# VainF/Diff-Pruning

Measured on NVIDIA H100. Metric: taylor_score_unet_fwd_bwd_passes_per_sec, higher is better.
Workload: dtype f32

## Files before the change

diff-pruning_b200/_lib.py:

```python
from __future__ import annotations

import ctypes as C
import os

_HERE = os.path.dirname(os.path.abspath(__file__))
LIB_PATH = os.path.join(_HERE, "libdpb200.so")

i32, i64, f32, u64, vp = C.c_int32, C.c_int64, C.c_float, C.c_uint64, C.c_void_p


class ConvArgs(C.Structure):
    _fields_ = [(n, i32) for n in ("N", "H", "W", "C", "P", "Q", "K", "R", "S", "stride", "pad_t", "pad_l", "flags",
                                   "splits")] + [
        ("x", vp), ("ldx", i64), ("y", vp), ("ldy", i64), ("w", vp), ("w_tc_hi", vp), ("w_tc_lo", vp), ("bias", vp), ("rowadd", vp),
        ("ld_rowadd", i64), ("residual", vp), ("ld_res", i64), ("workspace", vp), ("amax_x", vp), ("amax_y", vp), ("amax_w", vp), ("amax_out", vp), ("bias_ws", vp)]


class WgradReduceArgs(C.Structure):
    _fields_ = [(n, i32) for n in ("K", "C", "R", "S", "splits")] + [
        ("workspace", vp), ("dw", vp), ("w", vp), ("score_out", vp), ("score_in", vp), ("bias_ws", vp), ("db", vp)]


class GemmArgs(C.Structure):
    _fields_ = [("M", i32), ("N", i32), ("Kd", i32), ("batch", i32),
                ("A", vp), ("a_rs", i64), ("a_cs", i64), ("a_bs", i64),
                ("B", vp), ("b_rs", i64), ("b_cs", i64), ("b_bs", i64),
                ("C", vp), ("ldc", i64), ("c_bs", i64), ("alpha", f32), ("accumulate", i32)]


class GemmNtArgs(C.Structure):
    _fields_ = [("batch", i32), ("H", i32), ("W", i32), ("Kg", i32), ("N", i32), ("A", vp), ("ld_a", i64), ("b_hi", vp),
                ("b_lo", vp), ("C", vp), ("ldc", i64), ("alpha", f32), ("amax_a", vp), ("amax_b", vp), ("amax_out", vp)]


class GnArgs(C.Structure):
    _fields_ = [("N", i32), ("HW", i32), ("C", i32), ("G", i32), ("eps", f32), ("silu", i32),
                ("x", vp), ("ldx", i64), ("y", vp), ("ldy", i64), ("gamma", vp), ("beta", vp), ("mean", vp),
                ("rstd", vp), ("dy", vp), ("lddy", i64), ("dx", vp), ("lddx", i64), ("dx_add", vp), ("ldadd", i64),
                ("dx_add2", vp), ("ldadd2", i64), ("dgamma", vp), ("dbeta", vp), ("workspace", vp),
                ("dropout_p", f32), ("dropout_seed", u64), ("dropout_seed_dev", vp), ("y_bf16", vp), ("ldyb", i64),
                ("amax_y", vp), ("amax_dx", vp), ("fin", vp)]


class ConvBf16Args(C.Structure):
    _fields_ = [(n, i32) for n in ("N", "H", "W", "C", "P", "Q", "K", "R", "S", "stride", "pad_t", "pad_l", "flags", "splits")] + [
        ("x_bf16", vp), ("ldx", i64), ("dy_bf16", vp), ("lddy", i64), ("out", vp), ("ld_out", i64), ("w_bf16", vp), ("bias", vp),
        ("rowadd", vp), ("ld_rowadd", i64), ("residual", vp), ("ld_res", i64), ("workspace", vp)]


class TaylorArgs(C.Structure):
    _fields_ = [("O", i32), ("I", i32), ("RS", i32), ("w", vp), ("dw", vp), ("out_signed", vp), ("out_abs", vp),
                ("out_sq", vp), ("in_signed", vp), ("in_abs", vp), ("in_sq", vp)]


class SsimArgs(C.Structure):
    _fields_ = [("x", vp), ("y", vp), ("format", i32), ("N", i32), ("C", i32), ("H", i32), ("W", i32), ("win_size", i32),
                ("win", C.c_double * 11), ("c1", C.c_double), ("c2", C.c_double), ("ssim_nc", vp), ("sse_n", vp)]


class AdamArgs(C.Structure):
    _fields_ = [("n", i64), ("p", vp), ("g", vp), ("m", vp), ("v", vp), ("ema", vp), ("sumsq", vp),
                ("max_norm", C.c_double), ("lr", C.c_double), ("beta1", C.c_double), ("beta2", C.c_double),
                ("eps", C.c_double), ("ema_decay", C.c_double),
                ("step", i32), ("grad_scale", f32), ("step_scalars", vp)]


_SIGS = {
    "dp_version": (C.c_int, []),
    "dp_strerror": (C.c_char_p, [C.c_int]),
    "dp_last_cuda_error": (C.c_int, []),
    "dp_launch_count": (i64, []),
    "dp_tc_available": (C.c_int, []),
    "dp_tc_weight_row": (C.c_int, [C.c_int]),
    "dp_conv2d_fprop": (C.c_int, [C.POINTER(ConvArgs), vp]),
    "dp_conv2d_dgrad": (C.c_int, [C.POINTER(ConvArgs), vp]),
    "dp_conv2d_wgrad": (C.c_int, [C.POINTER(ConvArgs), vp]),
    "dp_conv_splitk_workspace_floats": (i64, [C.POINTER(ConvArgs), C.c_int]),
    "dp_conv2d_wgrad_reduce": (C.c_int, [C.POINTER(WgradReduceArgs), vp]),
    "dp_pack_conv_weight": (C.c_int, [vp, i32, i32, i32, i32, vp, vp, vp]),
    "dp_pack_conv_weight_tc": (C.c_int, [vp, i32, i32, i32, i32, vp, vp, vp, vp, vp, vp]),
    "dp_amax": (C.c_int, [vp, i64, i64, i32, vp, vp]),
    "dp_zero_u32": (C.c_int, [vp, i64, vp]),
    "dp_bf16_available": (C.c_int, []),
    "dp_bf16_weight_row": (C.c_int, [C.c_int]),
    "dp_bf16_wgrad_ctile": (C.c_int, [C.c_int]),
    "dp_conv2d_fprop_bf16": (C.c_int, [C.POINTER(ConvBf16Args), vp]),
    "dp_conv2d_dgrad_bf16": (C.c_int, [C.POINTER(ConvBf16Args), vp]),
    "dp_conv2d_wgrad_bf16": (C.c_int, [C.POINTER(ConvBf16Args), vp]),
    "dp_conv_bf16_eligible": (C.c_int, [C.POINTER(ConvBf16Args), C.c_int]),
    "dp_cvt_bf16": (C.c_int, [vp, i64, i64, i32, vp, i64, vp]),
    "dp_pack_conv_weight_bf16": (C.c_int, [vp, i32, i32, i32, i32, vp, vp, vp]),
    "dp_gemm_batched": (C.c_int, [C.POINTER(GemmArgs), vp]),
    "dp_gemm_nt_tc": (C.c_int, [C.POINTER(GemmNtArgs), vp]),
    "dp_split_h3": (C.c_int, [vp, i64, i64, i32, i32, i32, i32, vp, vp, vp, vp]),
    "dp_transpose_batched": (C.c_int, [vp, vp, i32, i32, i32, vp]),
    "dp_softmax_fwd": (C.c_int, [vp, vp, i64, i32, vp]),
    "dp_softmax_bwd": (C.c_int, [vp, vp, vp, i64, i32, vp, vp]),
    "dp_groupnorm_workspace_bytes": (C.c_size_t, [i32, i32, i32, i32]),
    "dp_groupnorm_fwd": (C.c_int, [C.POINTER(GnArgs), vp]),
    "dp_groupnorm_bwd": (C.c_int, [C.POINTER(GnArgs), vp]),
    "dp_groupnorm_bwd_param": (C.c_int, [C.POINTER(GnArgs), vp]),
    "dp_silu_fwd": (C.c_int, [vp, vp, i64, vp]),
    "dp_silu_bwd": (C.c_int, [vp, vp, vp, i64, i32, vp]),
    "dp_geglu_fwd": (C.c_int, [vp, i64, vp, i64, i64, i32, vp]),
    "dp_geglu_bwd": (C.c_int, [vp, i64, vp, i64, vp, i64, i64, i32, vp]),
    "dp_timestep_embedding": (C.c_int, [vp, vp, vp, i32, i32, i32, vp]),
    "dp_add_noise": (C.c_int, [vp, vp, vp, vp, vp, i32, i32, i32, i32, i32, i64, vp]),
    "dp_nchw_to_nhwc": (C.c_int, [vp, vp, i64, i32, i32, i32, i32, vp]),
    "dp_nhwc_to_nchw": (C.c_int, [vp, i64, vp, i32, i32, i32, i32, i32, vp]),
    "dp_mse_partials": (i64, [i64]),
    "dp_mse_loss_grad": (C.c_int, [vp, vp, vp, i64, f32, f32, vp, vp, vp]),
    "dp_upsample2x_fwd": (C.c_int, [vp, i64, vp, i64, i32, i32, i32, i32, vp]),
    "dp_upsample2x_bwd": (C.c_int, [vp, i64, vp, i64, i32, i32, i32, i32, i32, vp]),
    "dp_colsum": (C.c_int, [vp, i64, i64, i32, i64, vp, i64, i32, vp]),
    "dp_add_views": (C.c_int, [vp, i64, vp, i64, vp, i64, i64, i32, vp]),
    "dp_copy_rows": (C.c_int, [vp, i64, vp, i64, i64, i32, vp]),
    "dp_taylor_reduce": (C.c_int, [C.POINTER(TaylorArgs), vp]),
    "dp_sumsq_partials": (i64, [i64]),
    "dp_sumsq": (C.c_int, [vp, i64, vp, vp, vp]),
    "dp_adam_clip_ema": (C.c_int, [C.POINTER(AdamArgs), vp]),
    "dp_ddim_step": (C.c_int, [vp, vp, vp, vp, i64, f32, f32, f32, f32, f32, f32, vp]),
    "dp_ddim_cfg_step": (C.c_int, [vp, i64, vp, vp, vp, vp, i64, vp, i32, i32, i32, i32, i32, f32, f32, f32, f32, f32, f32, vp]),
    "dp_scale": (C.c_int, [vp, i64, f32, vp]),
    "dp_fid_input": (C.c_int, [vp, i32, i32, i32, i32, i32, vp, i64, i32, i32, i32, i32, vp, vp]),
    "dp_pool3x3": (C.c_int, [vp, i64, vp, i64, i32, i32, i32, i32, i32, i32, i32, vp, vp]),
    "dp_global_mean": (C.c_int, [vp, i64, vp, i64, i32, i32, i32, i32, vp]),
    "dp_feature_moments": (C.c_int, [vp, i64, i64, i32, vp, vp, vp, vp]),
    "dp_ssim": (C.c_int, [C.POINTER(SsimArgs), vp]),
    "dp_vq_quantize": (C.c_int, [vp, i32, i32, i32, i32, f32, vp, i32, i32, vp, i64, vp, vp]),
    "dp_decode_images": (C.c_int, [vp, i64, i32, i32, i32, i32, vp, vp, vp]),
# ... 34 lines not shown
```

diff-pruning_b200/csrc/conv_tc.cu:

```cuda
#include <cuda.h>
#include <cuda_fp16.h>
#include "common.cuh"
#include "sm90.cuh"
#include "sm90_host.cuh"

namespace {
using namespace sm90;

constexpr int BM = 128, BK = 64;
constexpr int A_BYTES = BM * 32 * 4;

struct TcParams {
  int Nimg, H, W;
  int Nout;
  int kchunks;
  int bw, bh, bn, tiles_w, tiles_h;
  float* y; long long ldy;
  const float* bias;
  const float* rowadd; long long ld_rowadd;
  const float* residual; long long ld_res;
  int accumulate;
  int vec4;
  int ntaps;
  signed char dh[9], dw[9], wt[9];
  int os, oa, ob, Ho, Wo;
  int in_stride;
  float alpha;
  int b_from_img;
  const uint32_t* amax_a;
  const uint32_t* amax_b;
  uint32_t* amax_out;
  int ksplit, it_per_split;
  float* ws; long long ws_split_stride; int ws_ld;
  const float* gx; long long gldx;
  int gH, gW, gC, gQ, gPQ, gS, gstride, gpad_t, gpad_l, gM;
  int relu;
};

__device__ __forceinline__ int amax_exponent(const uint32_t* slot) {
  const int E = (int)((__ldg(slot) >> 23) & 0xFFu);
  return min(max(E, 14), 254);
}
__device__ __forceinline__ float scale_up(int E) { return __uint_as_float((uint32_t)(267 - E) << 23); }
__device__ __forceinline__ float scale_dn(int E) { return __uint_as_float((uint32_t)(E - 13) << 23); }
constexpr float LO_SCALE = 2048.f, LO_UNSCALE = 1.f / 2048.f;
__device__ __forceinline__ void split2(float a, float b, uint32_t& h, uint32_t& l) {
  const __half2 hh = __floats2half2_rn(a, b);
  const float2 hf = __half22float2(hh);
  const __half2 ll = __floats2half2_rn((a - hf.x) * LO_SCALE, (b - hf.y) * LO_SCALE);
  h = *reinterpret_cast<const uint32_t*>(&hh);
  l = *reinterpret_cast<const uint32_t*>(&ll);
}
__device__ __forceinline__ void split1(float v, __half& h, __half& l) {
  h = __float2half_rn(v);
  l = __float2half_rn((v - __half2float(h)) * LO_SCALE);
}

constexpr int PS_STAGES = 3, PS_BN = 128;
constexpr int PS_B_BYTES = PS_BN * BK * 2;
constexpr int PS_STAGE_BYTES = 2 * A_BYTES + 2 * PS_B_BYTES;

template <bool ANY>
__global__ void __launch_bounds__(THREADS, 1)
conv_tc_ps_kernel(const __grid_constant__ CUtensorMap mapA, const __grid_constant__ CUtensorMap mapBh,
                  const __grid_constant__ CUtensorMap mapBl, const TcParams p, const int tiles_m, const int total_tiles) {
  const int total_work = total_tiles * p.ksplit;
  extern __shared__ uint8_t smem_raw[];
  const uint32_t raw = smem_u32(smem_raw);
  const uint32_t pad_to = ((raw + 1023u) & ~1023u) - raw;
  uint8_t* smem = smem_raw + pad_to;
  const uint32_t sbase = raw + pad_to;
  const uint32_t bar0 = sbase + PS_STAGES * PS_STAGE_BYTES;
  auto full_bar = [&](int s) { return bar0 + 8u * s; };
  auto empty_bar = [&](int s) { return bar0 + 8u * (PS_STAGES + s); };
  const int wg = threadIdx.x >> 7, tid = threadIdx.x & 127;
  if (threadIdx.x == 0) {
    for (int s = 0; s < PS_STAGES; ++s) { mbar_init(full_bar(s), ANY ? 1 + 128 : 1); mbar_init(empty_bar(s), 8); }
    mbar_init_fence();
  }
  __syncthreads();
  const int iters_per_tile = p.ntaps * p.kchunks;

  auto tile_coords = [&](int tile, int& q0, int& p0, int& n0, int& nblk) {
    nblk = tile / tiles_m;
    const int tile_m = tile - nblk * tiles_m;
    const int tw = tile_m % p.tiles_w;
    const int th = (tile_m / p.tiles_w) % p.tiles_h;
    const int tn = tile_m / (p.tiles_w * p.tiles_h);
    q0 = tw * p.bw; p0 = th * p.bh; n0 = tn * p.bn;
  };

  if (wg == 0) {
    setmaxnreg_dec<40>();
    if constexpr (ANY) {
      const int t = threadIdx.x;
      if (t == 0) { prefetch_map(&mapBh); prefetch_map(&mapBl); }
      const uint32_t sw = (uint32_t)(t & 7);
      uint32_t g = 0;
      for (int wi = blockIdx.x; wi < total_work; wi += gridDim.x) {
        const int tile = wi % total_tiles, it0 = (wi / total_tiles) * p.it_per_split, it1 = min(iters_per_tile, it0 + p.it_per_split);
        const int nblk = tile / tiles_m, m = (tile - nblk * tiles_m) * BM + t;
        const bool mv = m < p.gM;
        const int n = mv ? m / p.gPQ : 0, rem = m - n * p.gPQ, pq = rem / p.gQ;
        const int hb = pq * p.gstride - p.gpad_t, wb = (rem - pq * p.gQ) * p.gstride - p.gpad_l;
        const float* xn = p.gx + (long long)n * p.gH * p.gW * p.gldx;
        for (int it = it0; it < it1; ++it, ++g) {
          const int s = g % PS_STAGES;
          const uint32_t ph = (g / PS_STAGES) & 1u;
          mbar_wait(empty_bar(s), ph ^ 1u);
          const int tap = it / p.kchunks, kc = it - tap * p.kchunks;
          const int r = tap / p.gS, h = hb + r, w = wb + (tap - r * p.gS);
          const uint32_t st = sbase + s * PS_STAGE_BYTES;
          if (t == 0) {
            mbar_expect_tx(full_bar(s), 2 * PS_B_BYTES);
            tma_load_3d(st + 2 * A_BYTES, &mapBh, full_bar(s), kc * BK, nblk * PS_BN, tap);
            tma_load_3d(st + 2 * A_BYTES + PS_B_BYTES, &mapBl, full_bar(s), kc * BK, nblk * PS_BN, tap);
          }
          const bool v = mv && h >= 0 && h < p.gH && w >= 0 && w < p.gW;
          const int cleft = v ? p.gC - kc * BK : 0;
          const float* src = v ? xn + ((long long)h * p.gW + w) * p.gldx + kc * BK : p.gx;
#pragma unroll
          for (int j = 0; j < 16; ++j) {
            const int nb = min(max(cleft - 4 * j, 0), 4) * 4;
            cp_async16(st + (j >> 3) * A_BYTES + t * 128 + ((((uint32_t)j & 7u) ^ sw) << 4), nb ? src + 4 * j : p.gx, (uint32_t)nb);
          }
          cp_async_mbar_arrive(full_bar(s));
        }
      }
      return;
    }
    if (threadIdx.x == 0) {
      prefetch_map(&mapA); prefetch_map(&mapBh); prefetch_map(&mapBl);
      uint32_t g = 0;
      for (int wi = blockIdx.x; wi < total_work; wi += gridDim.x) {
        const int tile = wi % total_tiles, it0 = (wi / total_tiles) * p.it_per_split, it1 = min(iters_per_tile, it0 + p.it_per_split);
        int q0, p0, n0, nblk;
        tile_coords(tile, q0, p0, n0, nblk);
        for (int it = it0; it < it1; ++it, ++g) {
          const int s = g % PS_STAGES;
          const uint32_t ph = (g / PS_STAGES) & 1u;
          mbar_wait(empty_bar(s), ph ^ 1u);
          mbar_expect_tx(full_bar(s), PS_STAGE_BYTES);
          const int tap = it / p.kchunks, kc = it - tap * p.kchunks;
          const uint32_t st = sbase + s * PS_STAGE_BYTES;
          const int aw = q0 * p.in_stride + p.dw[tap], ah = p0 * p.in_stride + p.dh[tap];
          tma_load_4d(st, &mapA, full_bar(s), kc * BK, aw, ah, n0);
          tma_load_4d(st + A_BYTES, &mapA, full_bar(s), kc * BK + 32, aw, ah, n0);
          const int tapb = p.b_from_img ? n0 : p.wt[tap];
          tma_load_3d(st + 2 * A_BYTES, &mapBh, full_bar(s), kc * BK, nblk * PS_BN, tapb);
          tma_load_3d(st + 2 * A_BYTES + PS_B_BYTES, &mapBl, full_bar(s), kc * BK, nblk * PS_BN, tapb);
        }
      }
    }
    return;
  }
  setmaxnreg_inc<232>();
  const int c = wg - 1;
  const int warp = tid >> 5, lane = tid & 31;
  const uint32_t frag_row = (uint32_t)(64 * c + 16 * warp + (lane >> 2)) * 128 + 8 * (lane & 1);
  const uint32_t fsw = (uint32_t)(lane >> 2), fj = (uint32_t)((lane & 3) >> 1);
  const float sa = scale_up(amax_exponent(p.amax_a));
  const float f1 = scale_dn(amax_exponent(p.amax_a)), f2 = scale_dn(amax_exponent(p.amax_b)) * p.alpha;
  auto fin = [&](float main, float corr) { return fmaf(corr, LO_UNSCALE, main) * f1 * f2; };
  float amax = 0.f;
  uint32_t g = 0;
  for (int wi = blockIdx.x; wi < total_work; wi += gridDim.x) {
    const int tile = wi % total_tiles, it0 = (wi / total_tiles) * p.it_per_split, it1 = min(iters_per_tile, it0 + p.it_per_split);
    float acc[64], cor[64];
    uint32_t fh[2][4], fl[2][4];
    int prev_s = 0;
    for (int it = it0; it < it1; ++it, ++g) {
      const int s = g % PS_STAGES;
      const uint32_t ph = (g / PS_STAGES) & 1u;
      mbar_wait(full_bar(s), ph);
      const uint8_t* stp = smem + s * PS_STAGE_BYTES + frag_row;
      const uint32_t bst = sbase + s * PS_STAGE_BYTES + 2 * A_BYTES;
#pragma unroll
      for (int k = 0; k < BK / 16; ++k) {
        uint32_t (&ah)[4] = fh[k & 1];
        uint32_t (&al)[4] = fl[k & 1];
        const uint8_t* a = stp + (k >> 1) * A_BYTES;
        const uint32_t pos = ((4u * (k & 1) + fj) ^ fsw) << 4;
        const float2 v0 = *reinterpret_cast<const float2*>(a + pos), v1 = *reinterpret_cast<const float2*>(a + 1024 + pos);
        const float2 v2 = *reinterpret_cast<const float2*>(a + (pos ^ 32u)), v3 = *reinterpret_cast<const float2*>(a + 1024 + (pos ^ 32u));
        split2(v0.x * sa, v0.y * sa, ah[0], al[0]);
        split2(v1.x * sa, v1.y * sa, ah[1], al[1]);
        split2(v2.x * sa, v2.y * sa, ah[2], al[2]);
        split2(v3.x * sa, v3.y * sa, ah[3], al[3]);
        const uint64_t b_hi = desc_k(bst + k * 32), b_lo = desc_k(bst + PS_B_BYTES + k * 32);
        const uint32_t first = (it > it0 || k > 0) ? 1u : 0u;
        wgmma_fence();
        wgmma_f16_n128_rs<0>(acc, ah, b_hi, first);
        wgmma_f16_n128_rs<0>(cor, ah, b_lo, first);
        wgmma_f16_n128_rs<0>(cor, al, b_hi, 1u);
        wgmma_commit();
        wgmma_wait<1>();
        if (k == 0 && it > it0 && lane == 0) mbar_arrive(empty_bar(prev_s));
      }
      prev_s = s;
    }
    wgmma_wait<0>();
    fence_regs(acc); fence_regs(cor);
    if (lane == 0) mbar_arrive(empty_bar(prev_s));

    int q0, p0, n0, nblk;
    tile_coords(tile, q0, p0, n0, nblk);
#pragma unroll
    for (int i = 0; i < 2; ++i) {
      const int row = 64 * c + 16 * warp + (lane >> 2) + 8 * i;
      const int cb = 2 * (lane & 3);
      if (p.ksplit > 1) {
        float* wrow = p.ws + (long long)(wi / total_tiles) * p.ws_split_stride + ((long long)(tile - nblk * tiles_m) * BM + row) * p.ws_ld + nblk * PS_BN;
#pragma unroll
        for (int j = 0; j < 16; ++j)
          *reinterpret_cast<float2*>(wrow + 8 * j + cb) =
              make_float2(fin(acc[4 * j + 2 * i], cor[4 * j + 2 * i]), fin(acc[4 * j + 2 * i + 1], cor[4 * j + 2 * i + 1]));
        continue;
      }
      const int w_l = row % p.bw, h_l = (row / p.bw) % p.bh, n_l = row / (p.bw * p.bh);
      const int img = n0 + n_l;
      if (img >= p.Nimg) continue;
      if constexpr (ANY) { if (q0 + w_l >= p.Wo) continue; }
      const long long m = ((long long)img * p.Ho + ((p0 + h_l) * p.os + p.oa)) * p.Wo + ((q0 + w_l) * p.os + p.ob);
// ... 240 lines not shown
#pragma unroll
    for (int k = 0; k < WG_KPIX / 16; ++k) {
      const uint64_t b_hi = desc_mn(st + 4 * WG_BLK + k * 2048, WG_BLK), b_lo = desc_mn(st + 6 * WG_BLK + k * 2048, WG_BLK);
      const uint32_t first = (it > 0 || k > 0) ? 1u : 0u;
      wgmma_f16_n128_rs<1>(acc, fah[k], b_hi, first);
      wgmma_f16_n128_rs<1>(cor, fah[k], b_lo, first);
      wgmma_f16_n128_rs<1>(cor, fal[k], b_hi, 1u);
    }
    wgmma_commit();
    wgmma_wait<1>();
    if (it > 0 && lane == 0) mbar_arrive(empty_bar(prev_s));
    prev_s = s;
  };
  uint32_t fah0[4][4], fal0[4][4], fah1[4][4], fal1[4][4];
  int it = 0;
  for (; it + 1 < num_iters; it += 2) {
    stage(fah0, fal0, it);
    stage(fah1, fal1, it + 1);
  }
  if (it < num_iters) stage(fah0, fal0, it);
  wgmma_wait<0>();
  fence_regs(acc); fence_regs(cor);
#pragma unroll
  for (int i = 0; i < 2; ++i) {
    bsum[i] += __shfl_xor_sync(0xffffffffu, bsum[i], 1);
    bsum[i] += __shfl_xor_sync(0xffffffffu, bsum[i], 2);
  }
  const float f1 = scale_dn(Ey), f2 = scale_dn(Ex);
  const long long TC_ = (long long)T * p.C;
#pragma unroll
  for (int i = 0; i < 2; ++i) {
    const int kout = kt * 128 + 64 * c + 16 * warp + (lane >> 2) + 8 * i;
    if (kout >= p.K) continue;
    if (p.bias_ws && tap == 0 && ct == 0 && (lane & 3) == 0) p.bias_ws[(long long)blockIdx.y * p.K + kout] = bsum[i];
    float* wrow = p.ws + ((long long)blockIdx.y * p.K + kout) * TC_ + (long long)tap * p.C;
#pragma unroll
    for (int j = 0; j < 16; ++j)
#pragma unroll
      for (int e = 0; e < 2; ++e) {
        const int col = ct * 128 + 8 * j + 2 * (lane & 3) + e;
        if (col < p.C) wrow[col] = num_iters ? fmaf(cor[4 * j + 2 * i + e], LO_UNSCALE, acc[4 * j + 2 * i + e]) * f1 * f2 : 0.f;
      }
  }
}

constexpr int PS_SMEM = PS_STAGES * PS_STAGE_BYTES + 2048;
constexpr int WG_SMEM = WG_STAGES * WG_STAGE_BYTES + 2048;

static int wrow(int c) { return c > 64 ? ((c + 63) & ~63) : ((c + 7) & ~7); }

int tc_init() {
  static const int ok = [] {
    const bool set = runtime().encode &&
        cudaFuncSetAttribute(conv_tc_ps_kernel<false>, cudaFuncAttributeMaxDynamicSharedMemorySize, PS_SMEM) == cudaSuccess &&
        cudaFuncSetAttribute(conv_tc_ps_kernel<true>, cudaFuncAttributeMaxDynamicSharedMemorySize, PS_SMEM) == cudaSuccess &&
        cudaFuncSetAttribute(wgrad_tc_kernel, cudaFuncAttributeMaxDynamicSharedMemorySize, WG_SMEM) == cudaSuccess;
    (void)cudaGetLastError();
    return set ? 1 : 0;
  }();
  return ok;
}

static int pick_ksplit(int tiles, int iters, int& it_per_split) {
  it_per_split = iters;
  const int sms = runtime().num_sms;
  if (tiles * 2 > sms || iters < 8) return 1;
  int ks = sms / tiles;
  if (ks > iters / 4) ks = iters / 4;
  if (ks > 16) ks = 16;
  if (ks < 2) return 1;
  it_per_split = (iters + ks - 1) / ks;
  return (iters + it_per_split - 1) / it_per_split;
}

struct TcPlan { int bw, bh, bn, tiles_w, tiles_h, tiles_m, n_tiles, ksplit, it_per_split; long long ws_floats; };
int plan_tc(const ConvGemm& g, bool flat, bool split, TcPlan& pl) {
  if (!tc_init()) return DP_ERR_UNSUPPORTED;
  if (flat) { pl.bw = BM; pl.bh = 1; pl.bn = 1; }
  else if (!pick_box(BM, g.H, g.W, pl.bw, pl.bh, pl.bn)) return DP_ERR_UNSUPPORTED;
  pl.tiles_w = (g.W + pl.bw - 1) / pl.bw; pl.tiles_h = g.H / pl.bh;
  pl.tiles_m = pl.tiles_w * pl.tiles_h * ((g.N + pl.bn - 1) / pl.bn);
  pl.n_tiles = (g.Nout + PS_BN - 1) / PS_BN;
  const int iters = g.taps.n * ((g.Kg + BK - 1) / BK);
  pl.ksplit = 1; pl.it_per_split = iters;
  if (split) pl.ksplit = pick_ksplit(pl.tiles_m * pl.n_tiles, iters, pl.it_per_split);
  pl.ws_floats = pl.ksplit > 1 ? (long long)pl.ksplit * pl.tiles_m * BM * pl.n_tiles * PS_BN : 0;
  return DP_OK;
}

struct TcLaunch {
  const float* act; long long ld_act; const uint32_t* amax_a;
  const void* w_hi; const void* w_lo; const uint32_t* amax_b; int T; int ldb = -1;
  float* out; long long ld_out;
  const float* bias = nullptr; const float* rowadd = nullptr; long long ld_rowadd = 0; const float* residual = nullptr; long long ld_res = 0;
  int accumulate = 0;
  float* ws = nullptr;
  uint32_t* amax_out = nullptr;
  float alpha = 1.0f;
  int b_from_img = 0;
  const dp_conv_args* gather = nullptr;
};

TcLaunch conv_launch(const dp_conv_args* a, bool dgrad) {
  TcLaunch l{};
  l.act = (const float*)(dgrad ? a->y : a->x); l.ld_act = dgrad ? a->ldy : a->ldx; l.amax_a = dgrad ? a->amax_y : a->amax_x;
  l.w_hi = a->w_tc_hi; l.w_lo = a->w_tc_lo; l.amax_b = a->amax_w; l.T = a->R * a->S;
  l.out = (float*)(dgrad ? a->x : a->y); l.ld_out = dgrad ? a->ldx : a->ldy;
  if (!dgrad) { l.bias = a->bias; l.rowadd = a->rowadd; l.ld_rowadd = a->ld_rowadd; l.residual = a->residual; l.ld_res = a->ld_res; }
  l.accumulate = (a->flags & DP_CONV_ACCUMULATE) ? 1 : 0;
  l.ws = a->workspace; l.amax_out = a->amax_out;
  return l;
}

int launch_tc(const ConvGemm& g, const TcLaunch& l, cudaStream_t st) {
  const bool any = l.gather != nullptr, split = l.ws && !l.b_from_img;
  TcPlan pl;
  if (plan_tc(g, any, split, pl) != DP_OK) return DP_ERR_UNSUPPORTED;
  if (!l.w_hi || !l.w_lo || !l.amax_a || !l.amax_b) return DP_ERR_UNSUPPORTED;
  if (l.ld_act % 4 || ((uintptr_t)l.act & 15) || ((uintptr_t)l.w_hi & 15) || ((uintptr_t)l.w_lo & 15)) return DP_ERR_UNSUPPORTED;
  if (l.b_from_img && pl.bn != 1) return DP_ERR_UNSUPPORTED;
  CUtensorMap mA, mBh, mBl;
  if (!any) {
    const int s = g.in_stride;
    const cuuint64_t Hin = (cuuint64_t)g.H * s, Win = (cuuint64_t)g.W * s;
    cuuint64_t dims[4] = {(cuuint64_t)g.Kg, Win, Hin, (cuuint64_t)g.N};
    cuuint64_t str[3] = {(cuuint64_t)l.ld_act * 4, Win * l.ld_act * 4, Hin * Win * l.ld_act * 4};
    cuuint32_t box[4] = {32u, (cuuint32_t)(pl.bw * s), (cuuint32_t)(pl.bh * s), (cuuint32_t)pl.bn};
    if (box[1] > 256 || box[2] > 256) return DP_ERR_UNSUPPORTED;
    if (!encode_map(&mA, CU_TENSOR_MAP_DATA_TYPE_FLOAT32, l.act, 4, dims, str, box, s)) return DP_ERR_UNSUPPORTED;
  }
  {
    const cuuint64_t Kp = (cuuint64_t)(l.ldb < 0 ? wrow(g.Kg) : l.ldb);
    if (Kp % 8) return DP_ERR_UNSUPPORTED;
    cuuint64_t dims[3] = {Kp, (cuuint64_t)g.Nout, (cuuint64_t)l.T};
    cuuint64_t str[2] = {Kp * 2, (cuuint64_t)g.Nout * Kp * 2};
    cuuint32_t box[3] = {(cuuint32_t)BK, (cuuint32_t)PS_BN, 1};
    if (!encode_map(&mBh, CU_TENSOR_MAP_DATA_TYPE_FLOAT16, l.w_hi, 3, dims, str, box) ||
        !encode_map(&mBl, CU_TENSOR_MAP_DATA_TYPE_FLOAT16, l.w_lo, 3, dims, str, box)) return DP_ERR_UNSUPPORTED;
  }
  TcParams p{};
  p.Nimg = g.N; p.H = g.H; p.W = g.W; p.Nout = g.Nout;
  p.ntaps = g.taps.n;
  for (int i = 0; i < 9; ++i) { p.dh[i] = g.taps.dh[i]; p.dw[i] = g.taps.dw[i]; p.wt[i] = g.taps.wt[i]; }
  p.os = g.os; p.oa = g.oa; p.ob = g.ob; p.Ho = g.Ho; p.Wo = g.Wo;
  p.alpha = l.alpha; p.b_from_img = l.b_from_img; p.in_stride = g.in_stride; p.amax_a = l.amax_a; p.amax_b = l.amax_b; p.amax_out = l.amax_out;
  p.kchunks = (g.Kg + BK - 1) / BK;
  p.bw = pl.bw; p.bh = pl.bh; p.bn = pl.bn; p.tiles_w = pl.tiles_w; p.tiles_h = pl.tiles_h;
  p.y = l.out; p.ldy = l.ld_out; p.bias = l.bias; p.rowadd = l.rowadd; p.ld_rowadd = l.ld_rowadd; p.residual = l.residual; p.ld_res = l.ld_res;
  p.accumulate = l.accumulate;
  p.vec4 = (al16(l.out, l.ld_out) && al16(l.bias, 0) && al16(l.rowadd, l.ld_rowadd) && al16(l.residual, l.ld_res)) ? 1 : 0;
  p.ksplit = pl.ksplit; p.it_per_split = pl.it_per_split;
  if (split) { p.ws = l.ws; p.ws_ld = pl.n_tiles * PS_BN; p.ws_split_stride = (long long)pl.tiles_m * BM * p.ws_ld; }
  if (any) {
    const dp_conv_args* a = l.gather;
    p.gx = l.act; p.gldx = l.ld_act; p.gH = a->H; p.gW = a->W; p.gC = a->C; p.gQ = a->Q; p.gPQ = a->P * a->Q; p.gS = a->S;
    p.gstride = a->stride; p.gpad_t = a->pad_t; p.gpad_l = a->pad_l; p.gM = g.W; p.relu = (a->flags & DP_CONV_RELU) ? 1 : 0;
  }
  const int sms = runtime().num_sms, total = pl.tiles_m * pl.n_tiles, work = total * p.ksplit, ctas = work < sms ? work : sms;
  if (any) conv_tc_ps_kernel<true><<<ctas, THREADS, PS_SMEM, st>>>(mBh, mBh, mBl, p, pl.tiles_m, total);
  else conv_tc_ps_kernel<false><<<ctas, THREADS, PS_SMEM, st>>>(mA, mBh, mBl, p, pl.tiles_m, total);
  if (p.ksplit > 1) {
    const int rc = dp_check_launch();
    if (rc) return rc;
    const long long items = (any ? (long long)g.W : (long long)pl.tiles_m * BM) * ((g.Nout + 3) / 4);
    long long blocks = (items + 255) / 256;
    if (blocks > sms * 8) blocks = sms * 8;
    if (any) splitk_flat_epilogue_kernel<<<(int)blocks, 256, 0, st>>>(p);
    else splitk_epilogue_kernel<<<(int)blocks, 256, 0, st>>>(p, pl.tiles_m);
  }
  return dp_check_launch();
}

__global__ void pack_tc_kernel(const float* __restrict__ w, int K, int C, int RS, int Cp, int Kp, __half* __restrict__ kc_hi,
                               __half* __restrict__ kc_lo, __half* __restrict__ ck_hi, __half* __restrict__ ck_lo,
                               const uint32_t* __restrict__ amax) {
  const float sw = scale_up(amax_exponent(amax));
  const long long na = (long long)RS * K * Cp, nb = (long long)RS * C * Kp;
  const long long total = na > nb ? na : nb;
  for (long long i = blockIdx.x * (long long)blockDim.x + threadIdx.x; i < total; i += (long long)gridDim.x * blockDim.x) {
    if (i < na && kc_hi) {
      int c = (int)(i % Cp); long long t = i / Cp; int k = (int)(t % K), tap = (int)(t / K);
      split1(c < C ? w[((long long)k * C + c) * RS + tap] * sw : 0.f, kc_hi[i], kc_lo[i]);
    }
    if (i < nb && ck_hi) {
      int k = (int)(i % Kp); long long t = i / Kp; int c = (int)(t % C), tap = (int)(t / C);
      split1(k < K ? w[((long long)k * C + c) * RS + tap] * sw : 0.f, ck_hi[i], ck_lo[i]);
    }
  }
}
__global__ void split_h3_rows_kernel(const float* __restrict__ x, long long ld, long long bs, int rows, int cols, int pitch, int vec,
                                     __half* __restrict__ hi, __half* __restrict__ lo, const uint32_t* __restrict__ amax) {
  const float sx = scale_up(amax_exponent(amax));
  const int groups = pitch >> 3;
  const long long total = (long long)rows * groups;
  const float* xb = x + (long long)blockIdx.y * bs;
  __half* hb = hi + (long long)blockIdx.y * rows * pitch;
  __half* lb = lo + (long long)blockIdx.y * rows * pitch;
  for (long long i = blockIdx.x * 256ll + threadIdx.x; i < total; i += (long long)gridDim.x * 256) {
    const long long r = i / groups;
    const int c0 = (int)(i - r * groups) << 3;
    const float* src = xb + r * ld + c0;
    float v[8];
    if (vec && c0 + 8 <= cols) {
      const float4 a = __ldg(reinterpret_cast<const float4*>(src)), b = __ldg(reinterpret_cast<const float4*>(src + 4));
      v[0] = a.x; v[1] = a.y; v[2] = a.z; v[3] = a.w; v[4] = b.x; v[5] = b.y; v[6] = b.z; v[7] = b.w;
    } else {
#pragma unroll
      for (int j = 0; j < 8; ++j) v[j] = (c0 + j < cols) ? __ldg(src + j) : 0.f;
    }
    uint4 h, l;
    split2(v[0] * sx, v[1] * sx, h.x, l.x); split2(v[2] * sx, v[3] * sx, h.y, l.y);
    split2(v[4] * sx, v[5] * sx, h.z, l.z); split2(v[6] * sx, v[7] * sx, h.w, l.w);
    *reinterpret_cast<uint4*>(hb + r * pitch + c0) = h;
// ... 187 lines not shown
  if (!tc_init()) return DP_ERR_UNSUPPORTED;
  if (!box_geometry(a) || a->splits < 1) return DP_ERR_UNSUPPORTED;
  if (a->ldx % 4 || a->ldy % 4 || ((uintptr_t)a->x & 15) || ((uintptr_t)a->y & 15)) return DP_ERR_UNSUPPORTED;
  int bw, bh, bn;
  if (!a->amax_x || !a->amax_y) return DP_ERR_UNSUPPORTED;
  if (!pick_box(WG_KPIX, a->P, a->Q, bw, bh, bn)) return DP_ERR_UNSUPPORTED;
  const int img_boxes = (a->N + bn - 1) / bn;
  CUtensorMap mDy, mX;
  {
    cuuint64_t dims[4] = {(cuuint64_t)a->K, (cuuint64_t)a->Q, (cuuint64_t)a->P, (cuuint64_t)a->N};
    cuuint64_t str[3] = {(cuuint64_t)a->ldy * 4, (cuuint64_t)a->Q * a->ldy * 4, (cuuint64_t)a->P * a->Q * a->ldy * 4};
    cuuint32_t box[4] = {32, (cuuint32_t)bw, (cuuint32_t)bh, (cuuint32_t)bn};
    if (!encode_map(&mDy, CU_TENSOR_MAP_DATA_TYPE_FLOAT32, a->y, 4, dims, str, box)) return DP_ERR_UNSUPPORTED;
  }
  {
    cuuint64_t dims[4] = {(cuuint64_t)a->C, (cuuint64_t)a->W, (cuuint64_t)a->H, (cuuint64_t)a->N};
    cuuint64_t str[3] = {(cuuint64_t)a->ldx * 4, (cuuint64_t)a->W * a->ldx * 4, (cuuint64_t)a->H * a->W * a->ldx * 4};
    cuuint32_t box[4] = {32, (cuuint32_t)(bw * a->stride), (cuuint32_t)(bh * a->stride), (cuuint32_t)bn};
    if (box[1] > 256 || box[2] > 256) return DP_ERR_UNSUPPORTED;
    if (!encode_map(&mX, CU_TENSOR_MAP_DATA_TYPE_FLOAT32, a->x, 4, dims, str, box, a->stride)) return DP_ERR_UNSUPPORTED;
  }
  WgParams p{};
  p.Nimg = a->N; p.H = a->P; p.W = a->Q; p.C = a->C; p.K = a->K; p.R = a->R; p.S = a->S; p.pad = a->pad_t; p.in_stride = a->stride;
  p.bw = bw; p.bh = bh; p.bn = bn; p.tiles_w = a->Q / bw; p.tiles_h = a->P / bh;
  p.total_chunks = p.tiles_w * p.tiles_h * img_boxes;
  p.amax_x = a->amax_x; p.amax_y = a->amax_y; p.bias_ws = a->bias_ws;
  p.chunks_per_split = (p.total_chunks + a->splits - 1) / a->splits;
  p.c_tiles = (a->C + 127) / 128;
  p.ws = a->workspace;
  const int k_tiles = (a->K + 127) / 128;
  dim3 grid((unsigned)(k_tiles * p.c_tiles * a->R * a->S), (unsigned)a->splits);
  wgrad_tc_kernel<<<grid, THREADS, WG_SMEM, (cudaStream_t)stream>>>(mDy, mX, p);
  return dp_check_launch();
}

extern "C" int dp_pack_conv_weight_tc(const float* w, int32_t K, int32_t C, int32_t R, int32_t S, void* kc_hi, void* kc_lo,
                                      void* ck_hi, void* ck_lo, uint32_t* amax_w, dp_stream_t stream) {
  DP_REQUIRE(w && amax_w, DP_ERR_NULL);
  DP_REQUIRE((kc_hi == nullptr) == (kc_lo == nullptr) && (ck_hi == nullptr) == (ck_lo == nullptr), DP_ERR_NULL);
  DP_REQUIRE(K > 0 && C > 0 && R > 0 && S > 0, DP_ERR_SHAPE);
  if (cudaMemsetAsync(amax_w, 0, sizeof(uint32_t), (cudaStream_t)stream) != cudaSuccess) return dp_check_launch();
  int rc = dp_amax(w, (int64_t)C * R * S, K, C * R * S, amax_w, stream);
  if (rc) return rc;
  const int Cp = wrow(C), Kp = wrow(K);
  long long total = (long long)R * S * ((long long)K * Cp > (long long)C * Kp ? (long long)K * Cp : (long long)C * Kp);
  int blocks = (int)((total + 255) / 256);
  if (blocks > runtime().num_sms * 16) blocks = runtime().num_sms * 16;
  pack_tc_kernel<<<blocks, 256, 0, (cudaStream_t)stream>>>(w, K, C, R * S, Cp, Kp, (__half*)kc_hi, (__half*)kc_lo, (__half*)ck_hi, (__half*)ck_lo,
                                                           amax_w);
  return dp_check_launch();
}

extern "C" int dp_tc_weight_row(int channels) { return channels > 0 ? wrow(channels) : 0; }
```

include/dpb200.h:

```cpp
#ifndef DPB200_H
#define DPB200_H
#include <stddef.h>
#include <stdint.h>

#ifdef __cplusplus
extern "C" {
#endif

typedef void* dp_stream_t;

enum {
  DP_OK = 0,
  DP_ERR_SHAPE = -1,
  DP_ERR_ALIGN = -2,
  DP_ERR_UNSUPPORTED = -3,
  DP_ERR_CUDA = -4,
  DP_ERR_NULL = -5
};

int dp_version(void);
const char* dp_strerror(int code);
int dp_last_cuda_error(void);
int64_t dp_launch_count(void);
int dp_tc_available(void);

#define DP_CONV_ACCUMULATE 1
#define DP_CONV_FORCE_SIMT 2
#define DP_CONV_RELU 4
#define DP_CONV_ANY_GEOMETRY 8

typedef struct dp_conv_args {
  int32_t N, H, W, C;
  int32_t P, Q, K;
  int32_t R, S, stride, pad_t, pad_l;
  int32_t flags;
  int32_t splits;
  void* x;
  int64_t ldx;
  void* y;
  int64_t ldy;
  const float* w;
  const void* w_tc_hi;
  const void* w_tc_lo;
  const float* bias;
  const float* rowadd;
  int64_t ld_rowadd;
  const float* residual;
  int64_t ld_res;
  float* workspace;
  const uint32_t* amax_x; const uint32_t* amax_y; const uint32_t* amax_w;
  uint32_t* amax_out;
  float* bias_ws;
} dp_conv_args;

int dp_conv2d_fprop(const dp_conv_args* a, dp_stream_t stream);
int dp_conv2d_dgrad(const dp_conv_args* a, dp_stream_t stream);
long long dp_conv_splitk_workspace_floats(const dp_conv_args* a, int op);
int dp_conv2d_wgrad(const dp_conv_args* a, dp_stream_t stream);

typedef struct dp_wgrad_reduce_args {
  int32_t K, C, R, S, splits;
  const float* workspace;
  float* dw;
  const float* w;
  float* score_out;
  float* score_in;
  const float* bias_ws;
  float* db;
} dp_wgrad_reduce_args;
int dp_conv2d_wgrad_reduce(const dp_wgrad_reduce_args* a, dp_stream_t stream);

int dp_pack_conv_weight(const float* w_oihw, int32_t K, int32_t C, int32_t R, int32_t S, float* w_ck, float* w_kc,
                        dp_stream_t stream);

int dp_tc_weight_row(int channels);
int dp_pack_conv_weight_tc(const float* w_oihw, int32_t K, int32_t C, int32_t R, int32_t S, void* kc_hi, void* kc_lo,
                           void* ck_hi, void* ck_lo, uint32_t* amax_w, dp_stream_t stream);
int dp_amax(const float* x, int64_t ld, int64_t rows, int32_t cols, uint32_t* slot, dp_stream_t stream);
int dp_zero_u32(uint32_t* p, int64_t n, dp_stream_t stream);

typedef struct dp_conv_bf16_args {
  int32_t N, H, W, C;
  int32_t P, Q, K;
  int32_t R, S, stride, pad_t, pad_l;
  int32_t flags;
  int32_t splits;
  const void* x_bf16; int64_t ldx;
  const void* dy_bf16; int64_t lddy;
  float* out; int64_t ld_out;
  const void* w_bf16;
  const float* bias; const float* rowadd; int64_t ld_rowadd; const float* residual; int64_t ld_res;
  float* workspace;
} dp_conv_bf16_args;
int dp_bf16_available(void);
int dp_bf16_weight_row(int channels);
int dp_bf16_wgrad_ctile(int in_channels);
int dp_conv2d_fprop_bf16(const dp_conv_bf16_args* a, dp_stream_t stream);
int dp_conv2d_dgrad_bf16(const dp_conv_bf16_args* a, dp_stream_t stream);
int dp_conv2d_wgrad_bf16(const dp_conv_bf16_args* a, dp_stream_t stream);
int dp_conv_bf16_eligible(const dp_conv_bf16_args* a, int op);
int dp_cvt_bf16(const float* src, int64_t ld, int64_t rows, int32_t C, void* dst, int64_t ld_dst, dp_stream_t stream);
int dp_pack_conv_weight_bf16(const float* w_oihw, int32_t K, int32_t C, int32_t R, int32_t S, void* kc, void* ck, dp_stream_t stream);

typedef struct dp_gemm_args {
  int32_t M, N, Kd, batch;
  const float* A; int64_t a_rs, a_cs, a_bs;
  const float* B; int64_t b_rs, b_cs, b_bs;
  float* C; int64_t ldc, c_bs;
  float alpha;
  int32_t accumulate;
// ... 145 lines not shown
```

Measured before the change: 23.75.

## Add halo-tile path for 3x3 stride-1 tensor-core convs reusing one input load across taps

Adds a HALO variant of the persistent tensor-core conv kernel. For 3x3 stride-1 convs it loads one (bw+2)x(bh+2) input halo per K-chunk via TMA into double-buffered shared memory, then walks all nine taps over it with per-tap offsets, instead of re-loading a shifted A tile for every tap. This cuts A-operand global/TMA traffic by up to roughly ninefold. The cost is more shared memory, a different tile-shape search and split-K granularity rounded to whole K-chunks. A runtime toggle and a query API are also added.

```diff
diff --git a/diff-pruning_b200/_lib.py b/diff-pruning_b200/_lib.py
--- a/diff-pruning_b200/_lib.py
+++ b/diff-pruning_b200/_lib.py
@@ -76,6 +76,8 @@
     "dp_conv2d_dgrad": (C.c_int, [C.POINTER(ConvArgs), vp]),
     "dp_conv2d_wgrad": (C.c_int, [C.POINTER(ConvArgs), vp]),
     "dp_conv_splitk_workspace_floats": (i64, [C.POINTER(ConvArgs), C.c_int]),
+    "dp_conv_tc_halo_box": (C.c_int, [C.POINTER(ConvArgs), C.c_int, C.POINTER(i32)]),
+    "dp_conv_tc_set_halo": (C.c_int, [C.c_int]),
     "dp_conv2d_wgrad_reduce": (C.c_int, [C.POINTER(WgradReduceArgs), vp]),
     "dp_pack_conv_weight": (C.c_int, [vp, i32, i32, i32, i32, vp, vp, vp]),
     "dp_pack_conv_weight_tc": (C.c_int, [vp, i32, i32, i32, i32, vp, vp, vp, vp, vp, vp]),
diff --git a/diff-pruning_b200/csrc/conv_tc.cu b/diff-pruning_b200/csrc/conv_tc.cu
--- a/diff-pruning_b200/csrc/conv_tc.cu
+++ b/diff-pruning_b200/csrc/conv_tc.cu
@@ -35,6 +35,8 @@
   const float* gx; long long gldx;
   int gH, gW, gC, gQ, gPQ, gS, gstride, gpad_t, gpad_l, gM;
   int relu;
+  int halo_box, halo_tx;
+  int hoff[9];
 };
 
 __device__ __forceinline__ int amax_exponent(const uint32_t* slot) {
@@ -60,22 +62,31 @@
 constexpr int PS_B_BYTES = PS_BN * BK * 2;
 constexpr int PS_STAGE_BYTES = 2 * A_BYTES + 2 * PS_B_BYTES;
 
-template <bool ANY>
+constexpr int HALO_STAGE_BYTES = 2 * PS_B_BYTES;
+constexpr int HALO_MAX_LINES = 256;
+constexpr int HALO_SMEM_MAX = 4 * HALO_MAX_LINES * 128 + PS_STAGES * HALO_STAGE_BYTES + 2048;
+
+template <bool ANY, bool HALO>
 __global__ void __launch_bounds__(THREADS, 1)
 conv_tc_ps_kernel(const __grid_constant__ CUtensorMap mapA, const __grid_constant__ CUtensorMap mapBh,
                   const __grid_constant__ CUtensorMap mapBl, const TcParams p, const int tiles_m, const int total_tiles) {
+  static_assert(!(ANY && HALO), "the halo path loads A by TMA");
   const int total_work = total_tiles * p.ksplit;
   extern __shared__ uint8_t smem_raw[];
   const uint32_t raw = smem_u32(smem_raw);
   const uint32_t pad_to = ((raw + 1023u) & ~1023u) - raw;
   uint8_t* smem = smem_raw + pad_to;
   const uint32_t sbase = raw + pad_to;
-  const uint32_t bar0 = sbase + PS_STAGES * PS_STAGE_BYTES;
+  const uint32_t wbase = HALO ? sbase + 4u * p.halo_box : sbase;
+  const uint32_t bar0 = HALO ? wbase + PS_STAGES * HALO_STAGE_BYTES : sbase + PS_STAGES * PS_STAGE_BYTES;
   auto full_bar = [&](int s) { return bar0 + 8u * s; };
   auto empty_bar = [&](int s) { return bar0 + 8u * (PS_STAGES + s); };
+  auto hfull_bar = [&](int h) { return bar0 + 8u * (2 * PS_STAGES + h); };
+  auto hempty_bar = [&](int h) { return bar0 + 8u * (2 * PS_STAGES + 2 + h); };
   const int wg = threadIdx.x >> 7, tid = threadIdx.x & 127;
   if (threadIdx.x == 0) {
     for (int s = 0; s < PS_STAGES; ++s) { mbar_init(full_bar(s), ANY ? 1 + 128 : 1); mbar_init(empty_bar(s), 8); }
+    if constexpr (HALO) for (int h = 0; h < 2; ++h) { mbar_init(hfull_bar(h), 1); mbar_init(hempty_bar(h), 8); }
     mbar_init_fence();
   }
   __syncthreads();
@@ -129,6 +140,34 @@
       }
       return;
     }
+    if constexpr (HALO) {
+      if (threadIdx.x == 0) {
+        prefetch_map(&mapA); prefetch_map(&mapBh); prefetch_map(&mapBl);
+        uint32_t g = 0, hg = 0;
+        for (int wi = blockIdx.x; wi < total_work; wi += gridDim.x) {
+          const int tile = wi % total_tiles, it0 = (wi / total_tiles) * p.it_per_split, it1 = min(iters_per_tile, it0 + p.it_per_split);
+          int q0, p0, n0, nblk;
+          tile_coords(tile, q0, p0, n0, nblk);
+          for (int kc = it0 / p.ntaps; kc < it1 / p.ntaps; ++kc, ++hg) {
+            const int h = hg & 1;
+            mbar_wait(hempty_bar(h), ((hg >> 1) & 1u) ^ 1u);
+            mbar_expect_tx(hfull_bar(h), 2 * p.halo_tx);
+            const uint32_t hs = sbase + 2u * h * p.halo_box;
+            tma_load_4d(hs, &mapA, hfull_bar(h), kc * BK, q0 - 1, p0 - 1, n0);
+            tma_load_4d(hs + p.halo_box, &mapA, hfull_bar(h), kc * BK + 32, q0 - 1, p0 - 1, n0);
+            for (int tap = 0; tap < p.ntaps; ++tap, ++g) {
+              const int s = g % PS_STAGES;
+              mbar_wait(empty_bar(s), ((g / PS_STAGES) & 1u) ^ 1u);
+              mbar_expect_tx(full_bar(s), HALO_STAGE_BYTES);
+              const uint32_t st = wbase + s * HALO_STAGE_BYTES;
+              tma_load_3d(st, &mapBh, full_bar(s), kc * BK, nblk * PS_BN, p.wt[tap]);
+              tma_load_3d(st + PS_B_BYTES, &mapBl, full_bar(s), kc * BK, nblk * PS_BN, p.wt[tap]);
+            }
+          }
+        }
+      }
+      return;
+    }
     if (threadIdx.x == 0) {
       prefetch_map(&mapA); prefetch_map(&mapBh); prefetch_map(&mapBl);
       uint32_t g = 0;
@@ -163,12 +202,65 @@
   const float f1 = scale_dn(amax_exponent(p.amax_a)), f2 = scale_dn(amax_exponent(p.amax_b)) * p.alpha;
   auto fin = [&](float main, float corr) { return fmaf(corr, LO_UNSCALE, main) * f1 * f2; };
   float amax = 0.f;
-  uint32_t g = 0;
+  int hl[2] = {0, 0};
+  if constexpr (HALO) {
+#pragma unroll
+    for (int i = 0; i < 2; ++i) {
+      const int row = 64 * c + 16 * warp + (lane >> 2) + 8 * i;
+      const int w_l = row % p.bw, h_l = (row / p.bw) % p.bh, n_l = row / (p.bw * p.bh);
+      hl[i] = (n_l * (p.bh + 2) + h_l + 1) * (p.bw + 2) + w_l + 1;
+    }
+  }
+  uint32_t g = 0, hg = 0;
   for (int wi = blockIdx.x; wi < total_work; wi += gridDim.x) {
     const int tile = wi % total_tiles, it0 = (wi / total_tiles) * p.it_per_split, it1 = min(iters_per_tile, it0 + p.it_per_split);
     float acc[64], cor[64];
     uint32_t fh[2][4], fl[2][4];
     int prev_s = 0;
+    if constexpr (HALO) {
+      bool first = true;
+      for (int kc = it0 / p.ntaps; kc < it1 / p.ntaps; ++kc, ++hg) {
+        const int h = hg & 1;
+        mbar_wait(hfull_bar(h), (hg >> 1) & 1u);
+        const uint8_t* hp = smem + 2 * h * p.halo_box + 8 * (lane & 1);
+        for (int tap = 0; tap < p.ntaps; ++tap, ++g) {
+          const int s = g % PS_STAGES;
+          mbar_wait(full_bar(s), (g / PS_STAGES) & 1u);
+          const int l0 = hl[0] + p.hoff[tap], l1 = hl[1] + p.hoff[tap];
+          const uint8_t* r0 = hp + l0 * 128;
+          const uint8_t* r1 = hp + l1 * 128;
+          const uint32_t sw0 = (uint32_t)(l0 & 7), sw1 = (uint32_t)(l1 & 7);
+          const uint32_t bst = wbase + s * HALO_STAGE_BYTES;
+#pragma unroll
+          for (int k = 0; k < BK / 16; ++k) {
+            uint32_t (&ah)[4] = fh[k & 1];
+            uint32_t (&al)[4] = fl[k & 1];
+            const int box = (k >> 1) * p.halo_box;
+            const uint32_t j = 4u * (k & 1) + fj;
+            const uint32_t pos0 = (j ^ sw0) << 4, pos1 = (j ^ sw1) << 4;
+            const float2 v0 = *reinterpret_cast<const float2*>(r0 + box + pos0), v1 = *reinterpret_cast<const float2*>(r1 + box + pos1);
+            const float2 v2 = *reinterpret_cast<const float2*>(r0 + box + (pos0 ^ 32u)), v3 = *reinterpret_cast<const float2*>(r1 + box + (pos1 ^ 32u));
+            split2(v0.x * sa, v0.y * sa, ah[0], al[0]);
+            split2(v1.x * sa, v1.y * sa, ah[1], al[1]);
+            split2(v2.x * sa, v2.y * sa, ah[2], al[2]);
+            split2(v3.x * sa, v3.y * sa, ah[3], al[3]);
+            const uint64_t b_hi = desc_k(bst + k * 32), b_lo = desc_k(bst + PS_B_BYTES + k * 32);
+            const uint32_t accum = (!first || k > 0) ? 1u : 0u;
+            wgmma_fence();
+            wgmma_f16_n128_rs<0>(acc, ah, b_hi, accum);
+            wgmma_f16_n128_rs<0>(cor, ah, b_lo, accum);
+            wgmma_f16_n128_rs<0>(cor, al, b_hi, 1u);
+            wgmma_commit();
+            wgmma_wait<1>();
+            if (k == 0 && !first && lane == 0) mbar_arrive(empty_bar(prev_s));
+          }
+          first = false;
+          prev_s = s;
+        }
+        __syncwarp();
+        if (lane == 0) mbar_arrive(hempty_bar(h));
+      }
+    } else
     for (int it = it0; it < it1; ++it, ++g) {
       const int s = g % PS_STAGES;
       const uint32_t ph = (g / PS_STAGES) & 1u;
@@ -515,8 +607,9 @@
 int tc_init() {
   static const int ok = [] {
     const bool set = runtime().encode &&
-        cudaFuncSetAttribute(conv_tc_ps_kernel<false>, cudaFuncAttributeMaxDynamicSharedMemorySize, PS_SMEM) == cudaSuccess &&
-        cudaFuncSetAttribute(conv_tc_ps_kernel<true>, cudaFuncAttributeMaxDynamicSharedMemorySize, PS_SMEM) == cudaSuccess &&
+        cudaFuncSetAttribute(conv_tc_ps_kernel<false, false>, cudaFuncAttributeMaxDynamicSharedMemorySize, PS_SMEM) == cudaSuccess &&
+        cudaFuncSetAttribute(conv_tc_ps_kernel<false, true>, cudaFuncAttributeMaxDynamicSharedMemorySize, HALO_SMEM_MAX) == cudaSuccess &&
+        cudaFuncSetAttribute(conv_tc_ps_kernel<true, false>, cudaFuncAttributeMaxDynamicSharedMemorySize, PS_SMEM) == cudaSuccess &&
         cudaFuncSetAttribute(wgrad_tc_kernel, cudaFuncAttributeMaxDynamicSharedMemorySize, WG_SMEM) == cudaSuccess;
     (void)cudaGetLastError();
     return set ? 1 : 0;
@@ -536,17 +629,42 @@
   return (iters + it_per_split - 1) / it_per_split;
 }
 
-struct TcPlan { int bw, bh, bn, tiles_w, tiles_h, tiles_m, n_tiles, ksplit, it_per_split; long long ws_floats; };
+bool halo_box(const ConvGemm& g, int& bw, int& bh, int& bn) {
+  if (g.taps.n != 9 || g.in_stride != 1 || g.os != 1) return false;
+  for (int i = 0; i < 9; ++i)
+    if (g.taps.dh[i] < -1 || g.taps.dh[i] > 1 || g.taps.dw[i] < -1 || g.taps.dw[i] > 1) return false;
+  int best = HALO_MAX_LINES + 1;
+  for (int w = BM; w >= 8; w /= 2) {
+    if (w > g.W || g.W % w) continue;
+    for (int h = 1; w * h <= BM; h *= 2) {
+      if (h > g.H || g.H % h) continue;
+      const int n = BM / (w * h);
+      if (n > 1 && h != g.H) continue;
+      const int lines = (w + 2) * (h + 2) * n;
+      if (lines < best) { best = lines; bw = w; bh = h; bn = n; }
+    }
+  }
+  return best <= HALO_MAX_LINES;
+}
+int halo_enabled = 1;
+
+struct TcPlan { int bw, bh, bn, tiles_w, tiles_h, tiles_m, n_tiles, ksplit, it_per_split; long long ws_floats; bool halo; };
 int plan_tc(const ConvGemm& g, bool flat, bool split, TcPlan& pl) {
   if (!tc_init()) return DP_ERR_UNSUPPORTED;
+  pl.halo = !flat && halo_enabled && halo_box(g, pl.bw, pl.bh, pl.bn);
   if (flat) { pl.bw = BM; pl.bh = 1; pl.bn = 1; }
-  else if (!pick_box(BM, g.H, g.W, pl.bw, pl.bh, pl.bn)) return DP_ERR_UNSUPPORTED;
+  else if (!pl.halo && !pick_box(BM, g.H, g.W, pl.bw, pl.bh, pl.bn)) return DP_ERR_UNSUPPORTED;
   pl.tiles_w = (g.W + pl.bw - 1) / pl.bw; pl.tiles_h = g.H / pl.bh;
   pl.tiles_m = pl.tiles_w * pl.tiles_h * ((g.N + pl.bn - 1) / pl.bn);
   pl.n_tiles = (g.Nout + PS_BN - 1) / PS_BN;
   const int iters = g.taps.n * ((g.Kg + BK - 1) / BK);
   pl.ksplit = 1; pl.it_per_split = iters;
   if (split) pl.ksplit = pick_ksplit(pl.tiles_m * pl.n_tiles, iters, pl.it_per_split);
+  if (pl.halo && pl.ksplit > 1) {
+    const int cps = (pl.it_per_split + g.taps.n - 1) / g.taps.n;
+    pl.it_per_split = cps * g.taps.n;
+    pl.ksplit = (iters / g.taps.n + cps - 1) / cps;
+  }
   pl.ws_floats = pl.ksplit > 1 ? (long long)pl.ksplit * pl.tiles_m * BM * pl.n_tiles * PS_BN : 0;
   return DP_OK;
 }
@@ -589,6 +707,7 @@
     cuuint64_t dims[4] = {(cuuint64_t)g.Kg, Win, Hin, (cuuint64_t)g.N};
     cuuint64_t str[3] = {(cuuint64_t)l.ld_act * 4, Win * l.ld_act * 4, Hin * Win * l.ld_act * 4};
     cuuint32_t box[4] = {32u, (cuuint32_t)(pl.bw * s), (cuuint32_t)(pl.bh * s), (cuuint32_t)pl.bn};
+    if (pl.halo) { box[1] = pl.bw + 2; box[2] = pl.bh + 2; }
     if (box[1] > 256 || box[2] > 256) return DP_ERR_UNSUPPORTED;
     if (!encode_map(&mA, CU_TENSOR_MAP_DATA_TYPE_FLOAT32, l.act, 4, dims, str, box, s)) return DP_ERR_UNSUPPORTED;
   }
@@ -619,9 +738,16 @@
     p.gx = l.act; p.gldx = l.ld_act; p.gH = a->H; p.gW = a->W; p.gC = a->C; p.gQ = a->Q; p.gPQ = a->P * a->Q; p.gS = a->S;
     p.gstride = a->stride; p.gpad_t = a->pad_t; p.gpad_l = a->pad_l; p.gM = g.W; p.relu = (a->flags & DP_CONV_RELU) ? 1 : 0;
   }
+  if (pl.halo) {
+    p.halo_tx = (pl.bw + 2) * (pl.bh + 2) * pl.bn * 128;
+    p.halo_box = (p.halo_tx + 1023) & ~1023;
+    for (int i = 0; i < 9; ++i) p.hoff[i] = g.taps.dh[i] * (pl.bw + 2) + g.taps.dw[i];
+  }
   const int sms = runtime().num_sms, total = pl.tiles_m * pl.n_tiles, work = total * p.ksplit, ctas = work < sms ? work : sms;
-  if (any) conv_tc_ps_kernel<true><<<ctas, THREADS, PS_SMEM, st>>>(mBh, mBh, mBl, p, pl.tiles_m, total);
-  else conv_tc_ps_kernel<false><<<ctas, THREADS, PS_SMEM, st>>>(mA, mBh, mBl, p, pl.tiles_m, total);
+  if (any) conv_tc_ps_kernel<true, false><<<ctas, THREADS, PS_SMEM, st>>>(mBh, mBh, mBl, p, pl.tiles_m, total);
+  else if (pl.halo)
+    conv_tc_ps_kernel<false, true><<<ctas, THREADS, 4 * p.halo_box + PS_STAGES * HALO_STAGE_BYTES + 2048, st>>>(mA, mBh, mBl, p, pl.tiles_m, total);
+  else conv_tc_ps_kernel<false, false><<<ctas, THREADS, PS_SMEM, st>>>(mA, mBh, mBl, p, pl.tiles_m, total);
   if (p.ksplit > 1) {
     const int rc = dp_check_launch();
     if (rc) return rc;
@@ -915,3 +1041,17 @@
 }
 
 extern "C" int dp_tc_weight_row(int channels) { return channels > 0 ? wrow(channels) : 0; }
+
+extern "C" int dp_conv_tc_halo_box(const dp_conv_args* a, int op, int32_t* box) {
+  if (!a || a->N <= 0 || a->H <= 0 || a->W <= 0 || !box_geometry(a) || (op == 0 && (a->flags & DP_CONV_RELU))) return 0;
+  ConvGemm g[4];
+  int bw, bh, bn;
+  if (conv_gemms(a, op, g) != 1 || !halo_box(g[0], bw, bh, bn)) return 0;
+  if (box) { box[0] = bw; box[1] = bh; box[2] = bn; }
+  return 1;
+}
+extern "C" int dp_conv_tc_set_halo(int enable) {
+  const int prev = halo_enabled;
+  halo_enabled = enable ? 1 : 0;
+  return prev;
+}
diff --git a/include/dpb200.h b/include/dpb200.h
--- a/include/dpb200.h
+++ b/include/dpb200.h
@@ -56,6 +56,8 @@
 int dp_conv2d_fprop(const dp_conv_args* a, dp_stream_t stream);
 int dp_conv2d_dgrad(const dp_conv_args* a, dp_stream_t stream);
 long long dp_conv_splitk_workspace_floats(const dp_conv_args* a, int op);
+int dp_conv_tc_halo_box(const dp_conv_args* a, int op, int32_t* box);
+int dp_conv_tc_set_halo(int enable);
 int dp_conv2d_wgrad(const dp_conv_args* a, dp_stream_t stream);
 
 typedef struct dp_wgrad_reduce_args {
```

Result: faster. 24.19 (median of 6 runs) (+1.8%).
